# EdwardsLabProjects/sequence-alignment-tools

Measured on AMD Instinct MI355X. Metric: Gbases/s scanned, 100k×20-mer primers k≤2, 3 Gbp DB at 1/2/4/8 GPUs, higher is better.
Workload: dtype u32

## Files before the change

### sequence-alignment-tools_amd/csrc/pm_bits.h

```cpp
#pragma once
#include <cstdint>
#include <utility>

#include <hip/hip_runtime.h>

namespace pm {

namespace {

template <int... Is, typename F>
__device__ __forceinline__ void static_each(std::integer_sequence<int, Is...>, F &&f) { (f(std::integral_constant<int, Is>()), ...); }
template <int N, typename F>
__device__ __forceinline__ void static_for(F &&f) { static_each(std::make_integer_sequence<int, N>(), f); }

template <int O>
__device__ __forceinline__ uint32_t bits_at(uint32_t w0) {
  static_assert(O >= 0 && O < 32, "offset");
  if constexpr (O == 0) return w0;
  else return w0 >> O;
}
template <int O, typename... W>
__device__ __forceinline__ uint32_t bits_at(uint32_t w0, uint32_t w1, W... more) {
  static_assert(O >= 0, "offset");
  if constexpr (O == 0) return w0;
  else if constexpr (O < 32) return __builtin_amdgcn_alignbit(w1, w0, O);
  else return bits_at<O - 32>(w1, more...);
}

template <bool NT = false>
__device__ __forceinline__ uint32_t load_packed(const uint32_t *packed, int64_t npacked, int64_t pos) {
  const int64_t i = pos >> 4;
  if (pos < 0 || i >= npacked) return 0u;
  return NT ? __builtin_nontemporal_load(packed + i) : packed[i];
}

}

}
```

### sequence-alignment-tools_amd/csrc/pm_pair.hip

```cpp
#include "pm_bits.h"
#include "pm_internal.h"
#include "pm_pair.h"
#include "pm_verify.h"
#include "pm_workmap.h"

#include <algorithm>
#include <cstring>
#include <thread>
#include <type_traits>
#include <utility>

namespace pm {

namespace {

constexpr int WAVES = PAIR_WAVES;
constexpr uint32_t F20 = 0xfffffu;
constexpr uint32_t WHAT_REST = 8u, WHAT_ALL = 16u;
__device__ __host__ __forceinline__ uint64_t slot_pack(uint32_t o1, uint32_t o2, uint32_t o3, bool walk) {
  return (uint64_t)o1 | ((uint64_t)o2 << 20) | ((uint64_t)o3 << 40) | ((uint64_t)(walk ? 8 : 0) << 60);
}

struct PairArgs {
  const uint8_t *text;
  int64_t n, begin, end;
  const uint32_t *packed;
  int64_t npacked;
  int64_t chunk0, chunk_len;
  int nchunks, ncombos, group;
  int work_map;
  int k, eos_code, debug;
  int stride;
  int fa[PAIR_MAX_COMBOS], fb[PAIR_MAX_COMBOS];
  const uint32_t *image;
  const uint2 *slots;
  const uint32_t *row_base;
  const uint32_t *first_pat, *order;
  const uint32_t *olist;
  uint32_t first_off[PAIR_MAX_COMBOS];
  uint32_t np;
  const uint2 *pat40;
  const uint8_t *pat_len;
  const uint32_t *pat_id;
  const uint8_t *pat_codes;
  const uint32_t *pat_zone;
  int viol_level;
  pm_hit *out;
  unsigned long long *counter;
  unsigned long long cap;
  uint4 *susp;
  unsigned long long *susp_count;
  unsigned long long susp_cap;
  uint64_t *seed_out;
  unsigned long long *seed_count;
  unsigned long long seed_cap;
  unsigned long long *stats;
};

typedef __attribute__((address_space(3))) uint32_t lds_u32;
typedef uint32_t u32x4 __attribute__((ext_vector_type(4)));
typedef uint32_t u32x2 __attribute__((ext_vector_type(2)));
typedef __attribute__((address_space(3))) u32x4 lds_u128;
__device__ __forceinline__ lds_u128 *lds128(uint32_t addr) { return reinterpret_cast<lds_u128 *>((uintptr_t)addr); }
__device__ __forceinline__ lds_u32 *lds32(uint32_t addr) { return reinterpret_cast<lds_u32 *>((uintptr_t)addr); }

__device__ __host__ __forceinline__ uint32_t field_of(uint64_t W, int j) { return (uint32_t)(W >> (10 * j)) & 0x3ffu; }
__device__ __host__ __forceinline__ void other_fields(int a, int b, int *c, int *d) {
  int o[2], t = 0;
  for (int j = 0; j < 4; ++j) if (j != a && j != b) o[t++] = j;
  *c = o[0]; *d = o[1];
}


template <int OFF>
__device__ __forceinline__ uint32_t wbits(uint32_t wlo, uint32_t whi) {
  static_assert(OFF >= 0 && OFF < 48, "window offset");
  if constexpr (OFF == 0) return wlo;
  else if constexpr (OFF < 32) return __builtin_amdgcn_alignbit(whi, wlo, OFF);
  else return whi >> (OFF - 32);
}
template <int NB, int T>
__device__ __forceinline__ uint32_t mism(uint32_t p, uint32_t wlo, uint32_t whi) {
  static_assert(T >= -2 && T + NB <= 22, "text base outside the window");
  const uint32_t x = p ^ wbits<2 * (T + 2)>(wlo, whi);
  return (x | (x >> 1)) & (NB == 5 ? 0x155u : 0x55555u);
}
enum { REG_L = 0, REG_M = 1, REG_R = 2 };
template <int NB>
__device__ __forceinline__ bool two_deletions(uint32_t lowm, uint32_t midm, uint32_t highm) {
  const int lo = __builtin_ctz(lowm | (1u << (2 * NB)));
  const int hi = 31 - __builtin_clz(highm | 1u);
  const uint32_t between = ((1u << hi) - 1u) & ~((2u << lo) - 1u);
  return (midm & between) == 0;
}
template <int KIND, int NB, int T0, int BASE, int DSP, int BUDGET>
__device__ __forceinline__ int region_cost(uint32_t p, uint32_t wlo, uint32_t whi) {
  const uint32_t m0 = mism<NB, T0 + BASE>(p, wlo, whi);
  if constexpr (KIND == REG_M) {
    if constexpr (DSP == 0) {
      int c = __popc(m0);
      if constexpr (BUDGET >= 2) {
        const int up = 1 + max(1, __popc(m0 & mism<NB, T0 + 1>(p, wlo, whi))), dn = 1 + max(1, __popc(m0 & mism<NB, T0 - 1>(p, wlo, whi)));
        c = min(c, min(up, dn));
      }
      return c;
    }
    else if constexpr (DSP == 1) return 1 + __popc(m0 & mism<NB, T0 - 1>(p, wlo, whi));
    else if constexpr (DSP == -1) return max(1, __popc(m0 & mism<NB, T0 + 1>(p, wlo, whi)));
    else if constexpr (DSP == 2) return 2 + __popc(m0 & mism<NB, T0 - 1>(p, wlo, whi) & mism<NB, T0 - 2>(p, wlo, whi));
    else return two_deletions<NB>(mism<NB, T0 + 2>(p, wlo, whi), mism<NB, T0 + 1>(p, wlo, whi), m0) ? 2 : 9;
  } else {
    int c = __popc(m0);
    if constexpr (BUDGET >= 1) {
      const uint32_t rp1 = mism<NB, T0 + BASE + 1>(p, wlo, whi), rn1 = mism<NB, T0 + BASE - 1>(p, wlo, whi);
      const uint32_t mp1 = m0 & rp1, mn1 = m0 & rn1;
      const int up = __popc(mp1), dn = __popc(mn1);
      c = min(c, KIND == REG_R ? min(1 + up, max(1, dn)) : min(max(1, up), 1 + dn));
      if constexpr (BUDGET >= 2) {
        const uint32_t rp2 = mism<NB, T0 + BASE + 2>(p, wlo, whi), rn2 = mism<NB, T0 + BASE - 2>(p, wlo, whi);
        if constexpr (KIND == REG_R) {
          const int ins2 = 2 + __popc(mp1 & rp2);
          c = min(c, min(ins2, two_deletions<NB>(m0, rn1, rn2) ? 2 : 9));
        } else {
          const int ins2 = 2 + __popc(mn1 & rn2);
          c = min(c, min(ins2, two_deletions<NB>(rp2, rp1, m0) ? 2 : 9));
        }
      }
    }
    return c;
  }
}
template <int A, int B, int DSP, bool LOOSE = false>
__device__ __forceinline__ int edit_cost(uint32_t o, uint32_t wlo, uint32_t whi) {
  constexpr int C = (A != 0 && B != 0) ? 0 : ((A != 1 && B != 1) ? 1 : 2);
  constexpr int D = (A != 3 && B != 3) ? 3 : ((A != 2 && B != 2) ? 2 : 1);
  constexpr int AD = DSP < 0 ? -DSP : DSP, BUD = 2 - AD;
  constexpr int BUD2 = LOOSE && DSP == 0 ? 1 : BUD;
  static_assert(B > A + 1 || DSP == 0, "adjacent key fields are not displaced");
  if constexpr (A == 0 && B == 1) return region_cost<REG_R, 10, 10, 0, 0, BUD>(o, wlo, whi);
  else if constexpr (A == 2 && B == 3) return region_cost<REG_L, 10, 0, 0, 0, BUD>(o, wlo, whi);
  else if constexpr (A == 0 && B == 3) return region_cost<REG_M, 10, 5, 0, DSP, BUD>(o, wlo, whi);
  else {
    int c1, c2;
    if constexpr (A == 1 && B == 2) {
      c1 = region_cost<REG_L, 5, 0, 0, 0, BUD2>(o, wlo, whi);
      c2 = region_cost<REG_R, 5, 15, 0, 0, BUD2>(o >> 10, wlo, whi);
    }
    else if constexpr (A == 0 && B == 2) {
      c1 = region_cost<REG_M, 5, 5, 0, DSP, BUD2>(o, wlo, whi);
      c2 = region_cost<REG_R, 5, 15, 0, 0, BUD2>(o >> 10, wlo, whi);
    }
    else {
      static_assert(A == 1 && B == 3 && C == 0 && D == 2, "fields");
      c1 = region_cost<REG_L, 5, 0, -DSP, 0, BUD2>(o, wlo, whi);
      c2 = region_cost<REG_M, 5, 10, 0, DSP, BUD2>(o >> 10, wlo, whi);
    }
    if constexpr (LOOSE && DSP == 0) return min(c1, c2) == 0 ? 0 : c1 + c2;
    else return c1 + c2;
  }
}
template <int A, int B, int DSP>
__device__ __forceinline__ uint32_t edit_key(uint32_t wlo, uint32_t whi) {
  return (wbits<4 + 10 * A - 2 * DSP>(wlo, whi) & 0x3ffu) | ((wbits<4 + 10 * B>(wlo, whi) & 0x3ffu) << 10);
}
template <typename F>
__device__ __forceinline__ void edit_variant(int v, F &&f) {
  using std::integral_constant;
  switch (v) {
    case 0: f(integral_constant<int, 0>(), integral_constant<int, 1>(), integral_constant<int, 0>()); break;
    case 1: f(integral_constant<int, 0>(), integral_constant<int, 2>(), integral_constant<int, -1>()); break;
    case 2: f(integral_constant<int, 0>(), integral_constant<int, 2>(), integral_constant<int, 0>()); break;
    case 3: f(integral_constant<int, 0>(), integral_constant<int, 2>(), integral_constant<int, 1>()); break;
    case 4: f(integral_constant<int, 0>(), integral_constant<int, 3>(), integral_constant<int, -2>()); break;
    case 5: f(integral_constant<int, 0>(), integral_constant<int, 3>(), integral_constant<int, -1>()); break;
    case 6: f(integral_constant<int, 0>(), integral_constant<int, 3>(), integral_constant<int, 0>()); break;
    case 7: f(integral_constant<int, 0>(), integral_constant<int, 3>(), integral_constant<int, 1>()); break;
    case 8: f(integral_constant<int, 0>(), integral_constant<int, 3>(), integral_constant<int, 2>()); break;
    case 9: f(integral_constant<int, 1>(), integral_constant<int, 2>(), integral_constant<int, 0>()); break;
    case 10: f(integral_constant<int, 1>(), integral_constant<int, 3>(), integral_constant<int, -1>()); break;
    case 11: f(integral_constant<int, 1>(), integral_constant<int, 3>(), integral_constant<int, 0>()); break;
    case 12: f(integral_constant<int, 1>(), integral_constant<int, 3>(), integral_constant<int, 1>()); break;
    case 13: f(integral_constant<int, 2>(), integral_constant<int, 3>(), integral_constant<int, 0>()); break;
    default: break;
  }
}
__device__ __host__ __forceinline__ int edit_variant_table(int var) { return var == 0 ? 0 : (var <= 3 ? 1 : (var <= 8 ? 2 : (var == 9 ? 3 : (var <= 12 ? 4 : 5)))); }


__device__ __forceinline__ void pair_resolve(const PairArgs &a, const VerifyStage &vs, int combo, uint32_t rank, uint32_t what, uint32_t wo, int64_t p, pm_hit *first, bool *have) {
  const uint32_t *fp = a.first_pat + a.first_off[combo];
  const uint32_t *ord = a.order + (size_t)combo * a.np;
  const uint32_t *ol = a.olist + (size_t)combo * a.np;
  const uint32_t t0 = fp[rank], t1 = fp[rank + 1];
  pm_hit hh;
  auto take = [&](bool ok) __attribute__((always_inline)) {
    const bool extra = ok && *have;
    if (ok && !*have) { *first = hh; *have = true; }
    pair_emit(a, vs, extra, hh);
  };
  for (uint32_t j = 0; j < 3; ++j)
    take(((what >> j) & 1u) && t0 + j < t1 && pair_verify<5>(a, combo, p, ord[t0 + j], &hh));
  if (what & (WHAT_REST | WHAT_ALL)) {
    for (uint32_t t = t0 + ((what & WHAT_ALL) ? 0u : 3u); t < t1; ++t)
      take(sym_distance(ol[t] ^ wo) <= a.k && pair_verify<5>(a, combo, p, ord[t], &hh));
  }
}

__global__ __launch_bounds__(256) void pm_pair_verify(PairArgs a) {
  unsigned long long n = *a.susp_count;
  if (n > a.susp_cap) n = a.susp_cap;
  verify_staged(a, n, [&](unsigned long long i, const VerifyStage &vs, pm_hit *first) __attribute__((always_inline)) {
    bool have = false;
    const uint4 r = a.susp[i];
    const uint64_t pw = ((uint64_t)r.w << 32) | r.z;
    if (r.x != 0xffffffffu) {
      const int combo = (int)((pw >> 40) & 7u);
      const uint32_t key = r.x, wo = r.y, row = key & 0x7fffu, bit = key >> 15;
      const uint32_t wd = a.image[(size_t)combo * PAIR_BITMAP_WORDS + row];
      if ((wd >> bit) & 1u) {
        const uint32_t lr = (uint32_t)__popc(wd & ((1u << bit) - 1u));
        const uint32_t rank = a.row_base[(size_t)combo * (PAIR_BITMAP_WORDS + 1) + row] + lr;
        uint32_t what = WHAT_ALL;
        if (lr < (uint32_t)a.stride - 1u) {
          const uint2 sl = a.slots[((size_t)combo * PAIR_BITMAP_WORDS + row) * (size_t)a.stride + lr];
          const uint64_t S = ((uint64_t)sl.y << 32) | sl.x;
          what = (sym_distance(((uint32_t)S ^ wo) & F20) <= a.k ? 1u : 0u) | (sym_distance(((uint32_t)(S >> 20) ^ wo) & F20) <= a.k ? 2u : 0u) |
                 (sym_distance(((uint32_t)(S >> 40) ^ wo) & F20) <= a.k ? 4u : 0u) | ((sl.y >> 31) ? WHAT_REST : 0u);
        }
        pair_resolve(a, vs, combo, rank, what, wo, (int64_t)(pw & 0xffffffffffull), first, &have);
      }
    }
    return have && !(a.debug & 16);
  });
}

template <int A, int B, int DSP = 0, int FLOOR = 0>
__device__ __forceinline__ void pair_scan_body(const PairArgs &a, const int combo, const int cj, const int variant = 0) {
  constexpr int C = (A != 0 && B != 0) ? 0 : ((A != 1 && B != 1) ? 1 : 2);
  constexpr int D = (A != 3 && B != 3) ? 3 : ((A != 2 && B != 2) ? 2 : 1);
  static_assert(A < B && C < D && C != A && C != B && D != A && D != B, "fields");
  const int lane = threadIdx.x & 63;
  const int wave = __builtin_amdgcn_readfirstlane((int)(threadIdx.x >> 6));
  const int64_t sub = a.chunk_len / WAVES;
  const int64_t ws = (a.chunk0 + cj) * a.chunk_len + (int64_t)wave * sub;
  int64_t own_lo = ws > a.begin ? ws : a.begin;
  int64_t own_hi = ws + sub;
  if (own_hi > a.end) own_hi = a.end;
  if (own_hi > a.n) own_hi = a.n;
  if (own_lo < 19) own_lo = 19;
  if (own_lo >= own_hi) return;

  const uint32_t stride = (uint32_t)a.stride, kmax = stride - 1u;
  const char *slots = reinterpret_cast<const char *>(a.slots + (size_t)combo * PAIR_BITMAP_WORDS * stride);
  uint32_t carry1, carry2;
  {
    const uint32_t pk = load_packed(a.packed, a.npacked, ws - 32 + 16 * (lane & 1));
    carry2 = __builtin_amdgcn_readlane(pk, 0);
    carry1 = __builtin_amdgcn_readlane(pk, 1);
  }
  const uint32_t QB = PAIR_BITMAP_WORDS * 4 + (uint32_t)wave * (PAIR_QUEUE * 16);
  int qn = 0;
  uint32_t keep = 0;

  const int64_t pre_hi = FLOOR == 3 ? own_hi + 1024 : own_hi;
  uint32_t q0 = load_packed(a.packed, a.npacked, ws + 16 * lane);
  uint32_t q1 = ws + 1024 < pre_hi ? load_packed(a.packed, a.npacked, ws + 1024 + 16 * lane) : 0u;
  uint32_t q2 = ws + 2048 < pre_hi ? load_packed(a.packed, a.npacked, ws + 2048 + 16 * lane) : 0u;
  uint32_t q3 = ws + 3072 < pre_hi ? load_packed(a.packed, a.npacked, ws + 3072 + 16 * lane) : 0u;
  const uint32_t *pk_wave = a.packed + (ws >> 4);
  uint32_t pf_idx = 4096u / 16u + (uint32_t)lane;

  const int negk1 = -(a.k + 1);

  unsigned long long blk_at = 0;
  uint32_t blk_left = 0, blk_next = 0;
  auto flush = [&]() __attribute__((always_inline)) {
    int done = 0;
    while (done < qn) {
      if (blk_left == 0) {
        const uint32_t want = max((uint32_t)(qn - done), blk_next);
        unsigned long long base = 0;
        if (lane == 0) base = atomicAdd(a.susp_count, (unsigned long long)want);
        blk_at = ((unsigned long long)__builtin_amdgcn_readfirstlane((uint32_t)(base >> 32)) << 32) | __builtin_amdgcn_readfirstlane((uint32_t)base);
        blk_left = want;
        blk_next = min(2u * max(want, 64u), 4096u);
      }
      const int take = min(qn - done, (int)blk_left);
      for (int e = lane; e < take; e += 64) {
        const u32x4 q = *lds128(QB + 16 * (uint32_t)(done + e));
        const uint64_t pw = (uint64_t)(ws + q.z) | ((uint64_t)(FLOOR == 3 ? variant : combo) << 40);
        if (blk_at + (unsigned long long)e < a.susp_cap) a.susp[blk_at + (unsigned long long)e] = make_uint4(q.x, q.y, (uint32_t)pw, (uint32_t)(pw >> 32));
      }
      blk_at += (unsigned long long)take; blk_left -= (uint32_t)take; done += take;
    }
    qn = 0;
  };
  auto give_back = [&]() __attribute__((always_inline)) {
    for (uint32_t e = (uint32_t)lane; e < blk_left; e += 64)
      if (blk_at + e < a.susp_cap) a.susp[blk_at + e] = make_uint4(0xffffffffu, 0xffffffffu, 0xffffffffu, 0xffffffffu);
    blk_left = 0;
  };
  auto enqueue = [&](bool mine, uint32_t key, uint32_t wo, uint32_t prel) __attribute__((always_inline)) {
    const unsigned long long bal = __ballot(mine);
    if (bal == 0) return;
    if (a.debug & 1) { keep ^= key; return; }
    if (mine) {
      const int s_ = qn + (int)__builtin_amdgcn_mbcnt_hi((uint32_t)(bal >> 32), __builtin_amdgcn_mbcnt_lo((uint32_t)bal, 0));
      u32x4 q;
      q.x = key; q.y = wo; q.z = prel; q.w = 0;
      *lds128(QB + 16 * (uint32_t)s_) = q;
    }
    qn += __popcll(bal);
    if (qn >= 64) flush();
  };

  auto key_of = [&](auto WIN, uint32_t prev2, uint32_t prev1, uint32_t cur) __attribute__((always_inline)) -> uint32_t {
    constexpr int I = decltype(WIN)::value;
    const uint32_t X = bits_at<2 * I + 26 + 10 * A - 2 - 2 * DSP>(prev2, prev1, cur);
    if constexpr (B == A + 1 && DSP == 0) return X;
    else { const uint32_t Y = bits_at<2 * I + 26 + 10 * B - 12>(prev2, prev1, cur); return (X & 0xffcu) | (Y & ~0xffcu); }
  };

#ifndef PM_PAIR_NR
#define PM_PAIR_NR 6
#endif
  constexpr int NR = PM_PAIR_NR;
  static_assert(NR % 2 == 0 && NR >= 4 && NR <= 12, "ring size");
  uint32_t P = 0;
  uint32_t pu1 = 0, pu2 = 0, pu3 = 0, cu1 = 0, cu2 = 0, cu3 = 0;
  uint32_t tagbase = 0xfffffff0u;
  u32x2 e_sl[NR];
  uint32_t e_key[NR], e_wo[NR], e_rel[NR], e_okm[NR], e_wd[NR];
  uint32_t e_hi[FLOOR >= 2 ? NR : 1];
  for (int d = 0; d < (FLOOR >= 2 ? NR : 1); ++d) e_hi[d] = 0;
#pragma unroll
  for (int d = 0; d < NR; ++d) { e_sl[d].x = 0; e_sl[d].y = 0; e_key[d] = e_wo[d] = e_rel[d] = e_okm[d] = e_wd[d] = 0; }
  uint32_t m5v, f20v, rowmask;
  asm volatile("v_mov_b32 %0, 0x55555\n v_mov_b32 %1, 0xfffff\n v_mov_b32 %2, 0x7fff" : "=v"(m5v), "=v"(f20v), "=v"(rowmask));

  auto round = [&](auto PHASE) __attribute__((always_inline)) {
    constexpr int PH = decltype(PHASE)::value, LD = (PH + NR - 1) % NR;
    if constexpr (FLOOR == 3) {
      const uint32_t lo = e_wo[PH], hi = e_hi[PH];
      const int d1 = edit_cost<A, B, DSP, true>(e_sl[PH].x & f20v, lo, hi) - 3;
      const int d2 = edit_cost<A, B, DSP, true>(__builtin_amdgcn_alignbit(e_sl[PH].y, e_sl[PH].x, 20) & f20v, lo, hi) - 3;
      const bool susp = (int)(((uint32_t)(d1 | d2) | e_sl[PH].y) & e_okm[PH]) < 0;
      enqueue(susp, lo, hi, ((e_rel[PH] >> 4) << 10) + 16u * (uint32_t)lane + (e_rel[PH] & 15u));
    } else if constexpr (FLOOR == 2) {
      constexpr int OC = 4 + 10 * C;
      const uint32_t lo = e_wo[PH], hi = e_hi[PH];
      uint32_t T[5];
      static_for<5>([&](auto SI) __attribute__((always_inline)) { constexpr int si = decltype(SI)::value; T[si] = __builtin_amdgcn_alignbit(hi, lo, OC + 2 * (si - 2)) & f20v; });
      auto score = [&](uint32_t o) __attribute__((always_inline)) -> int {
        uint32_t m[5];
        static_for<5>([&](auto SI) __attribute__((always_inline)) { constexpr int si = decltype(SI)::value; const uint32_t x = o ^ T[si]; m[si] = (x | (x >> 1)) & m5v; });
        const int c0 = __popc(m[2]), c1 = __popc(m[2] & m[3]) + 1, c1n = __popc(m[2] & m[1]) + 1;
        const int c2 = __popc(m[2] & m[3] & m[4]) + 2, c2n = __popc(m[2] & m[1] & m[0]) + 2;
        return min(min(c0, min(c1, c1n)), min(c2, c2n)) - 3;
      };
      const int d1 = score(e_sl[PH].x & f20v), d2 = score(__builtin_amdgcn_alignbit(e_sl[PH].y, e_sl[PH].x, 20) & f20v);
      const bool susp = (int)(((uint32_t)(d1 | d2) | e_sl[PH].y) & e_okm[PH]) < 0;
      enqueue(susp, e_key[PH], lo, ((e_rel[PH] >> 4) << 10) + 16u * (uint32_t)lane + (e_rel[PH] & 15u));
    } else {
      const uint32_t w = e_wo[PH];
      const uint32_t x1 = e_sl[PH].x ^ w, x2 = __builtin_amdgcn_alignbit(e_sl[PH].y, e_sl[PH].x, 20) ^ w, x3 = (e_sl[PH].y >> 8) ^ w;
      const int d1 = __popc((x1 | (x1 >> 1)) & m5v) + negk1;
      const int d2 = __popc((x2 | (x2 >> 1)) & m5v) + negk1;
      const int d3 = __popc((x3 | (x3 >> 1)) & m5v) + negk1;
      const bool susp = (int)(((uint32_t)(d1 | d2 | d3) | e_sl[PH].y) & e_okm[PH]) < 0;
      enqueue(susp, e_key[PH], w, ((e_rel[PH] >> 4) << 10) + 16u * (uint32_t)lane + (e_rel[PH] & 15u));
    }
    {
      const uint32_t bit = e_key[LD] >> 15;
      const uint32_t lr = min((uint32_t)__popc(__builtin_amdgcn_ubfe(e_wd[LD], 0, bit)), kmax);
      const uint32_t off = (__umul24(e_key[LD] & rowmask, stride) + lr) << 3;
      e_sl[LD] = *reinterpret_cast<const u32x2 *>(slots + off);
    }
    {
      uint32_t i;
      asm("v_ffbl_b32 %0, %1" : "=v"(i) : "v"(P));
      P &= P - 1u;
      const uint32_t okm = ~i;
      const bool cb = (i & 16u) != 0;
      const uint32_t j2 = i + i;
      const uint32_t u1 = cb ? cu1 : pu1, u2 = cb ? cu2 : pu2, u3 = cb ? cu3 : pu3;
      const uint32_t wlo = __builtin_amdgcn_alignbit(u2, u1, j2), whi = __builtin_amdgcn_alignbit(u3, u2, j2);
      auto from = [&](int O) __attribute__((always_inline)) -> uint32_t { return O == 0 ? wlo : (O == 10 ? wlo >> 10 : __builtin_amdgcn_alignbit(whi, wlo, 20)); };
      uint32_t key, wo;
      if constexpr (FLOOR != 0) {
        constexpr int OA = 4 + 10 * A - 2 * DSP, OB = 4 + 10 * B - 10, OCC = 4 + 10 * C, ODD = 4 + 10 * D - 10;
        key = (__builtin_amdgcn_alignbit(whi, wlo, OA) & 0x3ffu) | (__builtin_amdgcn_alignbit(whi, wlo, OB) & 0xffc00u);
        if constexpr (FLOOR >= 2) { wo = wlo; e_hi[PH] = whi; }
        else wo = (__builtin_amdgcn_alignbit(whi, wlo, OCC) & 0x3ffu) | (__builtin_amdgcn_alignbit(whi, wlo, ODD) & 0xffc00u);
      } else {
      if constexpr (B == A + 1) key = from(10 * A) & f20v; else key = (from(10 * A) & 0x3ffu) | (from(10 * B - 10) & 0xffc00u);
      if constexpr (D == C + 1) wo = from(10 * C) & f20v; else wo = (from(10 * C) & 0x3ffu) | (from(10 * D - 10) & 0xffc00u);
      }
      key &= (uint32_t)((int)okm >> 31);
      e_key[PH] = key; e_wo[PH] = wo; e_okm[PH] = okm;
      e_rel[PH] = tagbase + i;
      e_wd[PH] = *lds32((key & rowmask) << 2);
    }
  };
  int ph = 0;
  int quiet = NR + 1;
  auto two_rounds = [&]() __attribute__((always_inline)) {
    bool done = false;
    static_for<NR / 2>([&](auto Q) __attribute__((always_inline)) {
      constexpr int q = decltype(Q)::value;
      if (!done && ph == q) {
        round(std::integral_constant<int, 2 * q>()); round(std::integral_constant<int, 2 * q + 1>());
        ph = q + 1 == NR / 2 ? 0 : q + 1;
        done = true;
      }
    });
  };

  const bool stats = (a.debug & 32) != 0 && a.stats != nullptr;
  uint32_t st_blocks = 0, st_rounds = 0, st_hits = 0;
  int64_t bb = ws;
  const int rmin = (a.debug >> 8) & 15 ? (a.debug >> 8) & 15 : 2;
  while (bb < own_hi) {
    const uint32_t cur = q0;
    q0 = q1; q1 = q2; q2 = q3;
    if (bb + 4096 < pre_hi) q3 = pk_wave[pf_idx];
    pf_idx += 64u;
    const uint32_t prev1 = __builtin_amdgcn_update_dpp(carry1, cur, 0x138, 0xf, 0xf, false);
    const uint32_t prev2 = __builtin_amdgcn_update_dpp(carry2, prev1, 0x138, 0xf, 0xf, false);
    carry2 = __builtin_amdgcn_readlane(cur, 62);
    carry1 = __builtin_amdgcn_readlane(cur, 63);
    uint32_t own = 0xffffu;
    if (bb < own_lo || bb + 1024 > own_hi) {
      const int64_t pbase = bb + 16 * lane;
      const int64_t lo = own_lo - pbase, hi = own_hi - pbase;
      const uint32_t l = lo <= 0 ? 0u : (lo >= 16 ? 16u : (uint32_t)lo), hh = hi <= 0 ? 0u : (hi >= 16 ? 16u : (uint32_t)hi);
      own = ((1u << hh) - 1u) & ~((1u << l) - 1u);
    }
    uint32_t acc = 0;
    {
      uint32_t ks[16], wd[16];
      static_for<16>([&](auto WIN) __attribute__((always_inline)) {
        constexpr int I = decltype(WIN)::value;
        ks[I] = key_of(WIN, prev2, prev1, cur);
        wd[I] = *lds32(ks[I] & 0x1fffcu);
      });
      static_for<16>([&](auto WIN) __attribute__((always_inline)) {
        constexpr int I = decltype(WIN)::value;
        acc = __builtin_amdgcn_alignbit(wd[I] >> ((ks[I] >> 17) & 31u), acc, 1);
      });
    }
    P |= acc & (own << 16);
    if (stats) { st_hits += (uint32_t)__popc(acc & (own << 16)); ++st_blocks; }
    constexpr int WB = FLOOR != 0 ? 22 : 26;
    cu1 = __builtin_amdgcn_alignbit(prev1, prev2, WB); cu2 = __builtin_amdgcn_alignbit(cur, prev1, WB); cu3 = cur >> WB;
    if constexpr (FLOOR == 3) {
      const uint32_t nfirst = __builtin_amdgcn_readfirstlane(q0);
      const uint32_t nxt = __builtin_amdgcn_update_dpp(nfirst, cur, 0x130, 0xf, 0xf, false);
      cu3 |= nxt << 10;
    }
    if (__ballot(P != 0)) quiet = 0;
    if (quiet <= NR) {
      int r = 0;
      do { two_rounds(); r += 2; } while (r < rmin || __ballot((P & 0xffffu) != 0));
      quiet += r;
      st_rounds += (uint32_t)r;
    }
    P >>= 16; pu1 = cu1; pu2 = cu2; pu3 = cu3; tagbase += 16u;
    bb += 1024;
  }
  while (__ballot(P != 0)) two_rounds();
  for (int d = 0; d < NR / 2 + 1; ++d) two_rounds();
  if (keep == 0x9e3779b9u) a.susp[0] = make_uint4(keep, 0, 0, 0);
  flush();
  give_back();
  if (stats) {
    for (int o = 32; o > 0; o >>= 1) st_hits += (uint32_t)__shfl_xor((int)st_hits, o);
    if (lane == 0) { atomicAdd(a.stats, (unsigned long long)st_blocks); atomicAdd(a.stats + 1, (unsigned long long)st_rounds); atomicAdd(a.stats + 2, (unsigned long long)st_hits); }
  }
}

__device__ __forceinline__ bool pair_block_item(const PairArgs &a, int *combo, int *cj) {
  if (a.work_map == PAIR_MAP_XCD_SUPERCHUNK) pair_xcd_superchunk_item((int)blockIdx.x, a.nchunks, a.ncombos, a.group, combo, cj);
  else if (a.work_map == PAIR_MAP_XCD) pair_xcd_item((int)blockIdx.x, a.nchunks, a.ncombos, combo, cj);
  else pair_superchunk_item((int)blockIdx.x, a.nchunks, a.ncombos, a.group, combo, cj);
  return *cj < a.nchunks && *combo < a.ncombos;
}

__global__ __launch_bounds__(PAIR_THREADS) void pm_pair_scan(PairArgs a) {
  extern __shared__ uint32_t lds[];
  int combo, cj;
  if (!pair_block_item(a, &combo, &cj)) return;
  {
    const u32x4 *src = reinterpret_cast<const u32x4 *>(a.image + (size_t)combo * PAIR_BITMAP_WORDS);
    u32x4 *dst = reinterpret_cast<u32x4 *>(lds);
    for (int i = threadIdx.x; i < PAIR_BITMAP_WORDS / 4; i += PAIR_THREADS) dst[i] = src[i];
  }
  __syncthreads();
  const int fa = a.fa[combo], fb = a.fb[combo];
  switch (fa * 4 + fb) {
    case 1: pair_scan_body<0, 1>(a, combo, cj); break;
    case 2: pair_scan_body<0, 2>(a, combo, cj); break;
    case 3: pair_scan_body<0, 3>(a, combo, cj); break;
    case 6: pair_scan_body<1, 2>(a, combo, cj); break;
    case 7: pair_scan_body<1, 3>(a, combo, cj); break;
    case 11: pair_scan_body<2, 3>(a, combo, cj); break;
    default: break;
  }
}

template <int FLOOR>
__global__ __launch_bounds__(PAIR_THREADS) void pm_pair_edit_scan(PairArgs a) {
  extern __shared__ uint32_t lds[];
  int var, cj;
  if (!pair_block_item(a, &var, &cj)) return;
  const int table = edit_variant_table(var);
  {
    const u32x4 *src = reinterpret_cast<const u32x4 *>(a.image + (size_t)table * PAIR_BITMAP_WORDS);
    u32x4 *dst = reinterpret_cast<u32x4 *>(lds);
    for (int i = threadIdx.x; i < PAIR_BITMAP_WORDS / 4; i += PAIR_THREADS) dst[i] = src[i];
  }
  __syncthreads();
  switch (var) {
    case 0: pair_scan_body<0, 1, 0, FLOOR>(a, table, cj, 0); break;
    case 1: pair_scan_body<0, 2, -1, FLOOR>(a, table, cj, 1); break;
    case 2: pair_scan_body<0, 2, 0, FLOOR>(a, table, cj, 2); break;
    case 3: pair_scan_body<0, 2, 1, FLOOR>(a, table, cj, 3); break;
    case 4: pair_scan_body<0, 3, -2, FLOOR>(a, table, cj, 4); break;
    case 5: pair_scan_body<0, 3, -1, FLOOR>(a, table, cj, 5); break;
    case 6: pair_scan_body<0, 3, 0, FLOOR>(a, table, cj, 6); break;
    case 7: pair_scan_body<0, 3, 1, FLOOR>(a, table, cj, 7); break;
    case 8: pair_scan_body<0, 3, 2, FLOOR>(a, table, cj, 8); break;
    case 9: pair_scan_body<1, 2, 0, FLOOR>(a, table, cj, 9); break;
    case 10: pair_scan_body<1, 3, -1, FLOOR>(a, table, cj, 10); break;
    case 11: pair_scan_body<1, 3, 0, FLOOR>(a, table, cj, 11); break;
    case 12: pair_scan_body<1, 3, 1, FLOOR>(a, table, cj, 12); break;
    case 13: pair_scan_body<2, 3, 0, FLOOR>(a, table, cj, 13); break;
    default: break;
  }
}

constexpr int ESTAGE = 2048;
constexpr int EWORK = 3072;
__global__ __launch_bounds__(256) void pm_pair_edit_resolve(PairArgs a) {
  __shared__ uint64_t s_rec[ESTAGE];
  __shared__ uint4 s_susp[256];
  __shared__ uint32_t s_work[EWORK];
  __shared__ uint32_t s_t0[256];
  __shared__ unsigned long long s_base;
  __shared__ uint32_t s_fill, s_valid, s_full, s_nwork;
  unsigned long long n = *a.susp_count;
  if (n > a.susp_cap) n = a.susp_cap;
  const unsigned long long stride = (unsigned long long)gridDim.x * blockDim.x;
  const int lane = threadIdx.x & 63;
  if (threadIdx.x == 0) { s_fill = 0; s_valid = (uint32_t)ESTAGE; s_nwork = 0; }
  __syncthreads();
  auto emit = [&](bool ok, uint64_t rec) __attribute__((always_inline)) {
    const unsigned long long bal = __ballot(ok);
    if (bal == 0) return;
    const int leader = __ffsll((long long)bal) - 1;
    const uint32_t cnt = (uint32_t)__popcll(bal), mine = (uint32_t)__popcll(bal & ((1ull << lane) - 1ull));
    uint32_t pos = 0;
    if (lane == leader) pos = atomicAdd(&s_fill, cnt);
    pos = __builtin_amdgcn_readlane(pos, leader);
    if (pos + cnt <= (uint32_t)ESTAGE) { if (ok) s_rec[pos + mine] = rec; return; }
    unsigned long long base = 0;
    if (lane == leader) { atomicMin(&s_valid, pos); base = atomicAdd(a.seed_count, (unsigned long long)cnt); }
    const uint32_t blo = __builtin_amdgcn_readlane((uint32_t)base, leader), bhi = __builtin_amdgcn_readlane((uint32_t)(base >> 32), leader);
    if (ok) { const unsigned long long o = (((unsigned long long)bhi << 32) | blo) + mine; if (o < a.seed_cap) a.seed_out[o] = rec; }
  };
  auto flush = [&]() __attribute__((always_inline)) {
    __syncthreads();
    const uint32_t cnt = min(s_fill, s_valid);
    __syncthreads();
    if (threadIdx.x == 0) { s_base = cnt ? atomicAdd(a.seed_count, (unsigned long long)cnt) : 0ull; s_fill = 0; s_valid = (uint32_t)ESTAGE; }
    __syncthreads();
    for (uint32_t i = threadIdx.x; i < cnt; i += blockDim.x) if (s_base + i < a.seed_cap) a.seed_out[s_base + i] = s_rec[i];
    __syncthreads();
  };
  auto item = [&](uint32_t wlo, uint32_t whi, int var, uint64_t pos40, uint32_t t, bool live) __attribute__((always_inline)) {
    bool ok = false;
    uint64_t rec = 0;
    if (live) {
      const int table = edit_variant_table(var);
      const uint32_t o = a.olist[(size_t)table * a.np + t];
      int c = 9;
      edit_variant(var, [&](auto A_, auto B_, auto D_) __attribute__((always_inline)) { c = edit_cost<decltype(A_)::value, decltype(B_)::value, decltype(D_)::value>(o, wlo, whi); });
      ok = c <= 2;
      if (ok) rec = ((uint64_t)a.order[(size_t)table * a.np + t] << 40) | pos40;
    }
    emit(ok, rec);
  };
  for (unsigned long long base = (unsigned long long)blockIdx.x * blockDim.x; base < n; base += stride) {
    const unsigned long long i = base + threadIdx.x;
    uint32_t t0 = 0, t1 = 0;
    uint4 r = make_uint4(0, 0, 0, 0xffffffffu);
    if (i < n) r = a.susp[i];
    if (r.w != 0xffffffffu) {
      const int var = (int)((r.w >> 8) & 15u);
      uint32_t key = 0;
      edit_variant(var, [&](auto A_, auto B_, auto D_) __attribute__((always_inline)) { key = edit_key<decltype(A_)::value, decltype(B_)::value, decltype(D_)::value>(r.x, r.y); });
      const int table = edit_variant_table(var);
      const uint32_t row = key & 0x7fffu, bit = key >> 15;
      const uint32_t wd = a.image[(size_t)table * PAIR_BITMAP_WORDS + row];
      if ((wd >> bit) & 1u) {
        const uint32_t rank = a.row_base[(size_t)table * (PAIR_BITMAP_WORDS + 1) + row] + (uint32_t)__popc(wd & ((1u << bit) - 1u));
        const uint32_t *fp = a.first_pat + a.first_off[table];
        t0 = fp[rank]; t1 = fp[rank + 1];
      }
    }
    s_susp[threadIdx.x] = r;
    s_t0[threadIdx.x] = t0;
    const uint32_t len = t1 - t0;
    uint32_t at = len ? atomicAdd(&s_nwork, len) : 0u;
    uint32_t q = 0;
    for (; q < len && at + q < (uint32_t)EWORK; ++q) s_work[at + q] = ((uint32_t)threadIdx.x << 24) | q;
    __syncthreads();
    const uint32_t nw = min(s_nwork, (uint32_t)EWORK);
    for (uint32_t w0 = 0; w0 < nw; w0 += blockDim.x) {
      const uint32_t w = w0 + threadIdx.x;
      const bool live = w < nw;
      const uint32_t it = live ? s_work[w] : 0u;
      const uint4 sr = s_susp[it >> 24];
      item(sr.x, sr.y, (int)((sr.w >> 8) & 15u), ((uint64_t)(sr.w & 0xffu) << 32) | sr.z, s_t0[it >> 24] + (it & 0xffffffu), live);
    }
    {
      uint32_t t = t0 + q;
      while (__ballot(t < t1)) { item(r.x, r.y, (int)((r.w >> 8) & 15u), ((uint64_t)(r.w & 0xffu) << 32) | r.z, t, t < t1); if (t < t1) ++t; }
    }
    __syncthreads();
    if (threadIdx.x == 0) { s_full = s_fill > (uint32_t)(ESTAGE - 1024); s_nwork = 0; }
    __syncthreads();
    if (s_full) flush();
  }
  flush();
}

}


std::string pair_build(const std::vector<Pattern> &pats, const std::vector<uint32_t> &ids, const Alphabet &alpha, int k,
                       int eos_code, PairTables *out, int stride_knob, int slot_patterns) {
  const size_t SP = slot_patterns == 2 ? 2 : 3;
  PairTables &t = *out;
  t = PairTables();
  if (k < 1 || k > 2) return "the pair plan is built for k = 1 and k = 2";
  const bool norm = alpha.nch['A'] == 0 && alpha.nch['C'] == 1 && alpha.nch['G'] == 2 && alpha.nch['T'] == 3;
  const bool ascii = alpha.size == 256 && alpha.nch['A'] == 'A' && alpha.nch['C'] == 'C' && alpha.nch['G'] == 'G' && alpha.nch['T'] == 'T';
  if (!norm && !ascii) return "stream alphabet is neither A,C,G,T-normalized nor raw ASCII";
  t.ascii = ascii && !norm;
  t.k = k;
  t.eos_code = (eos_code >= 0 && eos_code < 256) ? eos_code : -1;
  auto base2 = [&](unsigned char ch) -> int {
    switch (ch) { case 'A': return 0; case 'C': return 1; case 'G': return t.ascii ? 3 : 2; case 'T': return t.ascii ? 2 : 3; }
    return -1;
  };
  const size_t np = pats.size();
  if (np == 0) return "no patterns";
  if (np >= ((size_t)1 << 30)) return "too many patterns";
  t.pat40.resize(np); t.pat_len.resize(np); t.pat_id.resize(np); t.pat_codes.assign(np * 32, 0); t.pat_zone.assign(np, 0);
  for (size_t j = 0; j < np; ++j) {
    const std::string &s = pats[j].s;
    const int L = (int)s.size();
    if (L < 20 || L > 32) return "the pair plan needs patterns of 20..32 characters";
    uint64_t w = 0;
    for (int i = 0; i < 20; ++i) {
      const int b2 = base2((unsigned char)s[L - 20 + i]);
      if (b2 < 0) return "pattern with characters other than A,C,G,T";
      w |= (uint64_t)b2 << (2 * i);
    }
    for (int i = 0; i < L; ++i) {
      if (base2((unsigned char)s[i]) < 0) return "pattern with characters other than A,C,G,T";
      t.pat_codes[j * 32 + i] = (uint8_t)alpha.nch[(unsigned char)s[i]];
    }
    t.pat40[j] = w; t.pat_len[j] = (uint8_t)L; t.pat_id[j] = ids[j];
    {
      const int es = std::max(0, std::min(L, pats[j].esb)), ee = std::max(0, std::min(L, pats[j].eeb));
      uint32_t z = 0;
      for (int i = 0; i < L; ++i) if (i < es || i >= L - ee) z |= 1u << i;
      t.pat_zone[j] = z;
    }
    t.maxlen = std::max(t.maxlen, L);
  }
  if (k == 1) { t.ncombos = 2; t.fa[0] = 0; t.fb[0] = 1; t.fa[1] = 2; t.fb[1] = 3; }
  else { t.ncombos = 0; for (int x = 0; x < 4; ++x) for (int y = x + 1; y < 4; ++y) { t.fa[t.ncombos] = x; t.fb[t.ncombos] = y; ++t.ncombos; } }
  const int C = t.ncombos;
  t.stride = stride_knob >= 2 && stride_knob <= 33 ? stride_knob : (np <= 230000 ? 12 : (np <= 300000 ? 14 : 16));
  const size_t ST = (size_t)t.stride, KMAX = ST - 1;
  t.image.assign((size_t)C * PAIR_BITMAP_WORDS, 0);
  t.order.assign((size_t)C * np, 0);
  t.olist.assign((size_t)C * np, 0);
  t.slots.assign((size_t)C * PAIR_BITMAP_WORDS * ST, 0);
  t.row_base.assign((size_t)C * (PAIR_BITMAP_WORDS + 1), 0);
  std::vector<std::vector<uint32_t>> fp(C);
  auto build_combo = [&](int ci) {
    const int fa = t.fa[ci], fb = t.fb[ci];
    int fc, fd;
    other_fields(fa, fb, &fc, &fd);
    std::vector<uint64_t> srt(np);
    for (size_t j = 0; j < np; ++j) {
      const uint32_t key = field_of(t.pat40[j], fa) | (field_of(t.pat40[j], fb) << 10);
      const uint32_t bitpos = ((key & 0x7fffu) << 5) | (key >> 15);
      srt[j] = ((uint64_t)bitpos << 32) | (uint64_t)j;
    }
    std::sort(srt.begin(), srt.end());
    uint32_t *img = &t.image[(size_t)ci * PAIR_BITMAP_WORDS];
    uint32_t *ord = &t.order[(size_t)ci * np];
    uint32_t *ol = &t.olist[(size_t)ci * np];
    uint64_t *slot = &t.slots[(size_t)ci * PAIR_BITMAP_WORDS * ST];
    uint32_t *rb = &t.row_base[(size_t)ci * (PAIR_BITMAP_WORDS + 1)];
    std::vector<uint32_t> &f = fp[ci];
    f.reserve(np + 1);
    for (size_t r = 0; r < (size_t)PAIR_BITMAP_WORDS; ++r) slot[r * ST + KMAX] = slot_pack(0, 0, 0, true);
    uint32_t cur_row = 0, in_row = 0;
    for (size_t j = 0; j < np;) {
      const uint32_t bitpos = (uint32_t)(srt[j] >> 32);
      size_t j2 = j;
      while (j2 < np && (uint32_t)(srt[j2] >> 32) == bitpos) ++j2;
      const uint32_t row = bitpos >> 5;
      while (cur_row < row) { rb[++cur_row] = (uint32_t)f.size(); in_row = 0; }
      img[row] |= 1u << (bitpos & 31u);
      f.push_back((uint32_t)j);
      uint32_t o[3] = {0, 0, 0};
      for (size_t q = j; q < j2; ++q) {
        const uint32_t pi = (uint32_t)srt[q];
        ord[q] = pi;
        ol[q] = field_of(t.pat40[pi], fc) | (field_of(t.pat40[pi], fd) << 10);
        if (q - j < SP) o[q - j] = field_of(t.pat40[pi], fc) | (field_of(t.pat40[pi], fd) << 10);
      }
      for (size_t q = std::min(j2 - j, SP); q < 3; ++q) o[q] = o[0];
      if (in_row < KMAX) slot[(size_t)row * ST + in_row] = slot_pack(o[0], o[1], o[2], j2 - j > SP);
      ++in_row;
      j = j2;
    }
    while (cur_row < (uint32_t)PAIR_BITMAP_WORDS) rb[++cur_row] = (uint32_t)f.size();
    f.push_back((uint32_t)np);
  };
  if (np * (size_t)C < 20000) for (int ci = 0; ci < C; ++ci) build_combo(ci);
  else {
    std::vector<std::thread> th;
    for (int ci = 0; ci < C; ++ci) th.emplace_back([&, ci]() { build_combo(ci); });
    for (std::thread &x : th) x.join();
  }
  for (int ci = 0; ci < C; ++ci) {
    t.first_off[ci] = t.first_pat.size();
    t.first_pat.insert(t.first_pat.end(), fp[ci].begin(), fp[ci].end());
  }
  return "";
}

hipError_t pair_upload(const PairTables &t, PairDevice *d, hipStream_t st) {
  pair_free(d);
  d->k = t.k; d->maxlen = t.maxlen; d->ncombos = t.ncombos; d->eos_code = t.eos_code; d->ascii = t.ascii; d->np = t.pat40.size(); d->stride = t.stride;
  for (int c = 0; c < PAIR_MAX_COMBOS; ++c) { d->fa[c] = t.fa[c]; d->fb[c] = t.fb[c]; d->first_off[c] = t.first_off[c]; }
  auto up = [&](const void *src, size_t bytes, void **dst) -> hipError_t {
    hipError_t e = hipMalloc(dst, bytes ? bytes : 16);
    if (e != hipSuccess) return e;
    return bytes ? hipMemcpyAsync(*dst, src, bytes, hipMemcpyHostToDevice, st) : hipSuccess;
  };
  hipError_t e;
  if ((e = up(t.image.data(), t.image.size() * 4, (void **)&d->image)) != hipSuccess) return e;
  if ((e = up(t.slots.data(), t.slots.size() * 8, (void **)&d->slots)) != hipSuccess) return e;
  if ((e = up(t.row_base.data(), t.row_base.size() * 4, (void **)&d->row_base)) != hipSuccess) return e;
  if ((e = up(t.first_pat.data(), t.first_pat.size() * 4, (void **)&d->first_pat)) != hipSuccess) return e;
  if ((e = up(t.order.data(), t.order.size() * 4, (void **)&d->order)) != hipSuccess) return e;
  if ((e = up(t.olist.data(), t.olist.size() * 4, (void **)&d->olist)) != hipSuccess) return e;
  if ((e = up(t.pat40.data(), t.pat40.size() * 8, (void **)&d->pat40)) != hipSuccess) return e;
  if ((e = up(t.pat_len.data(), t.pat_len.size(), (void **)&d->pat_len)) != hipSuccess) return e;
  if ((e = up(t.pat_id.data(), t.pat_id.size() * 4, (void **)&d->pat_id)) != hipSuccess) return e;
  if ((e = up(t.pat_codes.data(), t.pat_codes.size(), (void **)&d->pat_codes)) != hipSuccess) return e;
  if ((e = up(t.pat_zone.data(), t.pat_zone.size() * 4, (void **)&d->pat_zone)) != hipSuccess) return e;
  hipFuncAttributes fa;
  if ((e = hipFuncGetAttributes(&fa, reinterpret_cast<const void *>(pm_pair_scan))) != hipSuccess) return e;
  if (fa.sharedSizeBytes != 0) return hipErrorInvalidConfiguration;
  if ((e = hipFuncSetAttribute(reinterpret_cast<const void *>(pm_pair_scan), hipFuncAttributeMaxDynamicSharedMemorySize, PAIR_LDS_BYTES)) != hipSuccess) return e;
  return hipStreamSynchronize(st);
}

void pair_free(PairDevice *d) {
  void *ptrs[] = {d->image, d->slots, d->row_base, d->first_pat, d->order, d->olist, d->pat_id, d->pat40, d->pat_len, d->pat_codes, d->pat_zone};
  for (void *p : ptrs) if (p) (void)hipFree(p);
  *d = PairDevice();
}

ScanGeometry pair_geometry(const PairDevice &d, int64_t begin, int64_t end) {
  ScanGeometry g;
  int64_t chunk = 1 << 19;
  const int64_t range = end - begin;
  if (range / ((int64_t)1 << 21) * d.ncombos >= 256 * 16) chunk = (int64_t)1 << 21;
  else if (range / ((int64_t)1 << 20) * d.ncombos >= 256 * 16) chunk = (int64_t)1 << 20;
  if (d.knobs.seed_chunk >= 1024 * WAVES) chunk = d.knobs.seed_chunk / (1024 * WAVES) * (1024 * WAVES);
  g.seg_len = chunk;
  const int64_t c_lo = begin / chunk, c_hi = end > begin ? (end - 1) / chunk : c_lo - 1;
  g.nseg = (int)(c_hi - c_lo + 1);
  g.threads = PAIR_THREADS;
  g.blocks = g.nseg * d.ncombos;
  g.work_map = g.nseg >= PAIR_XCD_MIN_CHUNKS ? PAIR_MAP_XCD_SUPERCHUNK : PAIR_MAP_SUPERCHUNK;
  if (d.knobs.pair_map >= 0) g.work_map = d.knobs.pair_map;
  return g;
}

hipError_t pair_launch(const PairDevice &d, const uint8_t *d_text, const uint32_t *d_packed, int64_t n, int64_t begin, int64_t end,
                       pm_hit *d_out, unsigned long long *d_counter, uint64_t cap, void *d_susp, unsigned long long *d_susp_count, uint64_t susp_cap,
                       hipStream_t st, ScanGeometry *geo_out, unsigned long long *d_stats, int floor_mode,
                       uint64_t *seed_out, unsigned long long *seed_count, uint64_t seed_cap) {
  if (!d_packed) return hipErrorInvalidValue;
  if (end > n) end = n;
  if (floor_mode && (d.k != 2 || d.ncombos != 6)) return hipErrorInvalidValue;
  if (floor_mode == 3 && (!seed_out || !seed_count)) return hipErrorInvalidValue;
  ScanGeometry g = pair_geometry(d, begin, end);
  if (floor_mode) {
    g.blocks = g.nseg * 14;
    if (d.knobs.pair_map < 0) g.work_map = PAIR_MAP_SUPERCHUNK;
  }
  if (geo_out) *geo_out = g;
  if (g.blocks <= 0 || d.np == 0) return hipSuccess;
  PairArgs a;
  memset(&a, 0, sizeof(a));
  a.text = d_text; a.n = n; a.begin = begin; a.end = end;
  a.packed = d_packed; a.npacked = (n + 15) / 16;
  a.chunk_len = g.seg_len; a.chunk0 = begin / g.seg_len; a.nchunks = g.nseg; a.ncombos = d.ncombos;
  a.group = 256;
  if (d.knobs.seed_group > 0) a.group = d.knobs.seed_group;
  a.work_map = g.work_map;
  a.k = d.k; a.eos_code = d.eos_code;
  a.debug = d.knobs.seed_debug;
  for (int c = 0; c < PAIR_MAX_COMBOS; ++c) { a.fa[c] = d.fa[c]; a.fb[c] = d.fb[c]; a.first_off[c] = (uint32_t)d.first_off[c]; }
  a.stride = d.stride;
  a.image = d.image; a.slots = reinterpret_cast<const uint2 *>(d.slots); a.row_base = d.row_base; a.first_pat = d.first_pat; a.order = d.order; a.olist = d.olist;
  a.np = (uint32_t)d.np;
  a.pat40 = reinterpret_cast<const uint2 *>(d.pat40); a.pat_len = d.pat_len; a.pat_id = d.pat_id; a.pat_codes = d.pat_codes; a.pat_zone = d.pat_zone; a.viol_level = d.viol_level;
  a.out = d_out; a.counter = d_counter; a.cap = cap;
  if (!d_susp || !d_susp_count) return hipErrorInvalidValue;
  a.susp = reinterpret_cast<uint4 *>(d_susp); a.susp_count = d_susp_count; a.susp_cap = susp_cap;
  a.stats = d_stats;
  a.seed_out = seed_out; a.seed_count = seed_count; a.seed_cap = seed_cap;
  if (floor_mode) {
    a.ncombos = 14;
    hipError_t fe;
    if (floor_mode == 1) {
      if ((fe = hipFuncSetAttribute(reinterpret_cast<const void *>(pm_pair_edit_scan<1>), hipFuncAttributeMaxDynamicSharedMemorySize, PAIR_LDS_BYTES)) != hipSuccess) return fe;
      hipLaunchKernelGGL(pm_pair_edit_scan<1>, dim3(g.blocks), dim3(PAIR_THREADS), PAIR_LDS_BYTES, st, a);
    } else if (floor_mode == 2) {
      if ((fe = hipFuncSetAttribute(reinterpret_cast<const void *>(pm_pair_edit_scan<2>), hipFuncAttributeMaxDynamicSharedMemorySize, PAIR_LDS_BYTES)) != hipSuccess) return fe;
      hipLaunchKernelGGL(pm_pair_edit_scan<2>, dim3(g.blocks), dim3(PAIR_THREADS), PAIR_LDS_BYTES, st, a);
    } else {
      if ((fe = hipFuncSetAttribute(reinterpret_cast<const void *>(pm_pair_edit_scan<3>), hipFuncAttributeMaxDynamicSharedMemorySize, PAIR_LDS_BYTES)) != hipSuccess) return fe;
      hipLaunchKernelGGL(pm_pair_edit_scan<3>, dim3(g.blocks), dim3(PAIR_THREADS), PAIR_LDS_BYTES, st, a);
      if ((fe = hipGetLastError()) != hipSuccess) return fe;
      hipLaunchKernelGGL(pm_pair_edit_resolve, dim3(16384), dim3(256), 0, st, a);
    }
    return hipGetLastError();
  }
  hipLaunchKernelGGL(pm_pair_scan, dim3(g.blocks), dim3(PAIR_THREADS), PAIR_LDS_BYTES, st, a);
  hipError_t ce = hipGetLastError();
  if (ce != hipSuccess) return ce;
  hipLaunchKernelGGL(pm_pair_verify, dim3(32768), dim3(256), 0, st, a);
  return hipGetLastError();
}

}
```

Baseline: 216.3.

## Restructure pair scan into a continuous round pipeline with a deeper text prefetch queue

Replaces the per-block loop, which dispatched two_rounds through a runtime phase switch, with a state machine. Verify rounds now run in a statically unrolled ring, and block boundaries (load next word, compute bitmap hits) are handled at ring edges, so the software pipeline of slot loads stays full across blocks and drain stages. The prefetch queue depth now scales with NR/2+1, and late-landing loads are joined into the queue through asm barriers. The aim is to remove phase-dispatch branching and pipeline bubbles at block transitions, at the cost of much more complex control flow and higher register pressure.

```diff
diff --git a/sequence-alignment-tools_amd/csrc/pm_bits.h b/sequence-alignment-tools_amd/csrc/pm_bits.h
--- a/sequence-alignment-tools_amd/csrc/pm_bits.h
+++ b/sequence-alignment-tools_amd/csrc/pm_bits.h
@@ -12,6 +12,10 @@
 __device__ __forceinline__ void static_each(std::integer_sequence<int, Is...>, F &&f) { (f(std::integral_constant<int, Is>()), ...); }
 template <int N, typename F>
 __device__ __forceinline__ void static_for(F &&f) { static_each(std::make_integer_sequence<int, N>(), f); }
+template <int... Is, typename F>
+__device__ __forceinline__ bool static_all_each(std::integer_sequence<int, Is...>, F &&f) { return (f(std::integral_constant<int, Is>()) && ...); }
+template <int N, typename F>
+__device__ __forceinline__ bool static_all(F &&f) { return static_all_each(std::make_integer_sequence<int, N>(), f); }
 
 template <int O>
 __device__ __forceinline__ uint32_t bits_at(uint32_t w0) {
diff --git a/sequence-alignment-tools_amd/csrc/pm_pair.hip b/sequence-alignment-tools_amd/csrc/pm_pair.hip
--- a/sequence-alignment-tools_amd/csrc/pm_pair.hip
+++ b/sequence-alignment-tools_amd/csrc/pm_pair.hip
@@ -263,12 +263,7 @@
   uint32_t keep = 0;
 
   const int64_t pre_hi = FLOOR == 3 ? own_hi + 1024 : own_hi;
-  uint32_t q0 = load_packed(a.packed, a.npacked, ws + 16 * lane);
-  uint32_t q1 = ws + 1024 < pre_hi ? load_packed(a.packed, a.npacked, ws + 1024 + 16 * lane) : 0u;
-  uint32_t q2 = ws + 2048 < pre_hi ? load_packed(a.packed, a.npacked, ws + 2048 + 16 * lane) : 0u;
-  uint32_t q3 = ws + 3072 < pre_hi ? load_packed(a.packed, a.npacked, ws + 3072 + 16 * lane) : 0u;
   const uint32_t *pk_wave = a.packed + (ws >> 4);
-  uint32_t pf_idx = 4096u / 16u + (uint32_t)lane;
 
   const int negk1 = -(a.k + 1);
 
@@ -374,6 +369,7 @@
       const uint32_t bit = e_key[LD] >> 15;
       const uint32_t lr = min((uint32_t)__popc(__builtin_amdgcn_ubfe(e_wd[LD], 0, bit)), kmax);
       const uint32_t off = (__umul24(e_key[LD] & rowmask, stride) + lr) << 3;
+      asm volatile("" : : "v"(e_sl[LD]));
       e_sl[LD] = *reinterpret_cast<const u32x2 *>(slots + off);
     }
     {
@@ -402,29 +398,36 @@
       e_wd[PH] = *lds32((key & rowmask) << 2);
     }
   };
-  int ph = 0;
   int quiet = NR + 1;
-  auto two_rounds = [&]() __attribute__((always_inline)) {
-    bool done = false;
-    static_for<NR / 2>([&](auto Q) __attribute__((always_inline)) {
-      constexpr int q = decltype(Q)::value;
-      if (!done && ph == q) {
-        round(std::integral_constant<int, 2 * q>()); round(std::integral_constant<int, 2 * q + 1>());
-        ph = q + 1 == NR / 2 ? 0 : q + 1;
-        done = true;
-      }
-    });
-  };
 
   const bool stats = (a.debug & 32) != 0 && a.stats != nullptr;
   uint32_t st_blocks = 0, st_rounds = 0, st_hits = 0;
   int64_t bb = ws;
   const int rmin = (a.debug >> 8) & 15 ? (a.debug >> 8) & 15 : 2;
-  while (bb < own_hi) {
-    const uint32_t cur = q0;
-    q0 = q1; q1 = q2; q2 = q3;
-    if (bb + 4096 < pre_hi) q3 = pk_wave[pf_idx];
-    pf_idx += 64u;
+  constexpr int PD = NR / 2 + 1;
+  uint32_t q[PD], land[NR / 2];
+  static_for<PD>([&](auto I) __attribute__((always_inline)) {
+    constexpr int i = decltype(I)::value;
+    q[i] = i == 0 || ws + 1024 * i < pre_hi ? load_packed(a.packed, a.npacked, ws + 1024 * i + 16 * lane) : 0u;
+  });
+  static_for<NR / 2>([&](auto I) __attribute__((always_inline)) { land[decltype(I)::value] = 0; });
+  int qfill = PD;
+  uint32_t landed = 0;
+  uint32_t pf_idx = (uint32_t)PD * 64u + (uint32_t)lane;
+  auto q_take = [&]() __attribute__((always_inline)) -> uint32_t {
+    const uint32_t cur = q[0];
+    static_for<PD - 1>([&](auto I) __attribute__((always_inline)) { constexpr int i = decltype(I)::value; q[i] = q[i + 1]; });
+    --qfill;
+    return cur;
+  };
+  auto q_join = [&](uint32_t w) __attribute__((always_inline)) {
+    static_for<PD>([&](auto I) __attribute__((always_inline)) {
+      constexpr int i = decltype(I)::value;
+      if (qfill == i) { const uint32_t from = w; uint32_t to; asm volatile("v_mov_b32 %0, %1" : "=v"(to) : "v"(from)); q[i] = to; }
+    });
+    ++qfill;
+  };
+  auto block_begin = [&](const uint32_t cur) __attribute__((always_inline)) {
     const uint32_t prev1 = __builtin_amdgcn_update_dpp(carry1, cur, 0x138, 0xf, 0xf, false);
     const uint32_t prev2 = __builtin_amdgcn_update_dpp(carry2, prev1, 0x138, 0xf, 0xf, false);
     carry2 = __builtin_amdgcn_readlane(cur, 62);
@@ -454,22 +457,69 @@
     constexpr int WB = FLOOR != 0 ? 22 : 26;
     cu1 = __builtin_amdgcn_alignbit(prev1, prev2, WB); cu2 = __builtin_amdgcn_alignbit(cur, prev1, WB); cu3 = cur >> WB;
     if constexpr (FLOOR == 3) {
-      const uint32_t nfirst = __builtin_amdgcn_readfirstlane(q0);
+      const uint32_t nfirst = __builtin_amdgcn_readfirstlane(q[0]);
       const uint32_t nxt = __builtin_amdgcn_update_dpp(nfirst, cur, 0x130, 0xf, 0xf, false);
       cu3 |= nxt << 10;
     }
-    if (__ballot(P != 0)) quiet = 0;
-    if (quiet <= NR) {
-      int r = 0;
-      do { two_rounds(); r += 2; } while (r < rmin || __ballot((P & 0xffffu) != 0));
-      quiet += r;
-      st_rounds += (uint32_t)r;
-    }
+  };
+  int r = 0;
+  int rlim = rmin;
+  int stage = 0;
+  auto block_end = [&]() __attribute__((always_inline)) {
+    quiet += r; if (stage == 0) st_rounds += (uint32_t)r;
     P >>= 16; pu1 = cu1; pu2 = cu2; pu3 = cu3; tagbase += 16u;
-    bb += 1024;
-  }
-  while (__ballot(P != 0)) two_rounds();
-  for (int d = 0; d < NR / 2 + 1; ++d) two_rounds();
+    bb += 1024; r = 0;
+  };
+  bool leave = false;
+  auto edge = [&](auto Q) __attribute__((always_inline)) -> bool {
+    constexpr int e = decltype(Q)::value;
+    if (e == 0 && leave) return false;
+    if (landed & (1u << e)) { q_join(land[e]); landed &= ~(1u << e); }
+    if (leave) return true;
+    if (r < rlim || __ballot((P & 0xffffu) != 0)) return true;
+    block_end();
+    if (bb < own_hi) {
+      const uint32_t cur = q_take();
+      if (bb + 1024 * PD < pre_hi) land[e] = pk_wave[pf_idx];
+      pf_idx += 64u; landed |= 1u << e;
+      block_begin(cur);
+      if (__ballot(P != 0)) quiet = 0;
+      leave = quiet > NR;
+    }
+    else if (stage == 0 && __ballot(P != 0)) { stage = 1; rlim = 0; }
+    else if (stage < 2) { stage = 2; rlim = NR; }
+    else { stage = 3; leave = true; }
+    return true;
+  };
+  while (stage < 3) {
+    for (;;) {
+      if (bb >= own_hi) { stage = 3; break; }
+      const uint32_t cur = q_take();
+      if (bb + 1024 * PD < pre_hi) q[PD - 1] = pk_wave[pf_idx];
+      pf_idx += 64u; ++qfill;
+      block_begin(cur);
+      if (__ballot(P != 0)) quiet = 0;
+      if (quiet <= NR) break;
+      block_end();
+    }
+    if (stage == 3) break;
+    leave = false;
+    { const uint32_t last = q[PD - 1]; asm volatile("" : : "v"(last)); }
+    while (static_all<NR / 2>([&](auto Q) __attribute__((always_inline)) {
+      constexpr int q2 = decltype(Q)::value;
+      if (!edge(Q)) return false;
+      round(std::integral_constant<int, 2 * q2>()); round(std::integral_constant<int, 2 * q2 + 1>());
+      r += 2;
+      return true;
+    })) {}
+    static_for<NR / 2>([&](auto E) __attribute__((always_inline)) {
+      constexpr int e = decltype(E)::value;
+      if (landed & (1u << e)) q_join(land[e]);
+    });
+    landed = 0;
+    r = 0;
+    if (stage < 3) block_end();
+  }
   if (keep == 0x9e3779b9u) a.susp[0] = make_uint4(keep, 0, 0, 0);
   flush();
   give_back();
```

Result: slower. 213.0 (-1.5%).

## Restructure scan loop into phase-unrolled ring state machine with unconditional prefetch

Applied to the files above, without the earlier changes.

Replaces the main scan loop, which dispatched on a runtime ring phase through two_rounds, with an unrolled for(;;) chain of per-phase macros. Each ring pair is compiled with a static phase, and new blocks are taken only when the ring is ready to advance. The prefetch load becomes unconditional, clamping its index to the lane instead of branching, and readfirstlane moves earlier. Both changes aim to remove per-round phase-selection branches and let loads overlap compute. The cost is larger code, goto-based control flow, and tail handling that relies on tagbase and P shift bookkeeping being kept exactly in step.

```diff
diff --git a/sequence-alignment-tools_amd/csrc/pm_pair.hip b/sequence-alignment-tools_amd/csrc/pm_pair.hip
--- a/sequence-alignment-tools_amd/csrc/pm_pair.hip
+++ b/sequence-alignment-tools_amd/csrc/pm_pair.hip
@@ -328,7 +328,7 @@
   static_assert(NR % 2 == 0 && NR >= 4 && NR <= 12, "ring size");
   uint32_t P = 0;
   uint32_t pu1 = 0, pu2 = 0, pu3 = 0, cu1 = 0, cu2 = 0, cu3 = 0;
-  uint32_t tagbase = 0xfffffff0u;
+  uint32_t tagbase = 0xffffffe0u;
   u32x2 e_sl[NR];
   uint32_t e_key[NR], e_wo[NR], e_rel[NR], e_okm[NR], e_wd[NR];
   uint32_t e_hi[FLOOR >= 2 ? NR : 1];
@@ -415,16 +415,25 @@
       }
     });
   };
-
   const bool stats = (a.debug & 32) != 0 && a.stats != nullptr;
   uint32_t st_blocks = 0, st_rounds = 0, st_hits = 0;
   int64_t bb = ws;
   const int rmin = (a.debug >> 8) & 15 ? (a.debug >> 8) & 15 : 2;
-  while (bb < own_hi) {
-    const uint32_t cur = q0;
-    q0 = q1; q1 = q2; q2 = q3;
-    if (bb + 4096 < pre_hi) q3 = pk_wave[pf_idx];
+
+  auto next_word = [&](uint32_t *nfirst) __attribute__((always_inline)) -> uint32_t {
+    uint32_t cur, n0, n1, n2;
+    asm volatile("v_mov_b32 %0, %4\n v_mov_b32 %1, %5\n v_mov_b32 %2, %6\n v_mov_b32 %3, %7"
+                 : "=&v"(cur), "=&v"(n0), "=&v"(n1), "=&v"(n2) : "v"(q0), "v"(q1), "v"(q2), "v"(q3));
+    q0 = n0; q1 = n1; q2 = n2;
+    q3 = pk_wave[bb + 4096 < pre_hi ? pf_idx : (uint32_t)lane];
     pf_idx += 64u;
+    if constexpr (FLOOR == 3) *nfirst = __builtin_amdgcn_readfirstlane(q0);
+    return cur;
+  };
+  auto take_block = [&]() __attribute__((always_inline)) {
+    P >>= 16; pu1 = cu1; pu2 = cu2; pu3 = cu3; tagbase += 16u;
+    uint32_t nfirst = 0;
+    const uint32_t cur = next_word(&nfirst);
     const uint32_t prev1 = __builtin_amdgcn_update_dpp(carry1, cur, 0x138, 0xf, 0xf, false);
     const uint32_t prev2 = __builtin_amdgcn_update_dpp(carry2, prev1, 0x138, 0xf, 0xf, false);
     carry2 = __builtin_amdgcn_readlane(cur, 62);
@@ -454,22 +463,46 @@
     constexpr int WB = FLOOR != 0 ? 22 : 26;
     cu1 = __builtin_amdgcn_alignbit(prev1, prev2, WB); cu2 = __builtin_amdgcn_alignbit(cur, prev1, WB); cu3 = cur >> WB;
     if constexpr (FLOOR == 3) {
-      const uint32_t nfirst = __builtin_amdgcn_readfirstlane(q0);
       const uint32_t nxt = __builtin_amdgcn_update_dpp(nfirst, cur, 0x130, 0xf, 0xf, false);
       cu3 |= nxt << 10;
     }
+    bb += 1024;
     if (__ballot(P != 0)) quiet = 0;
-    if (quiet <= NR) {
-      int r = 0;
-      do { two_rounds(); r += 2; } while (r < rmin || __ballot((P & 0xffffu) != 0));
-      quiet += r;
-      st_rounds += (uint32_t)r;
-    }
-    P >>= 16; pu1 = cu1; pu2 = cu2; pu3 = cu3; tagbase += 16u;
-    bb += 1024;
-  }
-  while (__ballot(P != 0)) two_rounds();
-  for (int d = 0; d < NR / 2 + 1; ++d) two_rounds();
+  };
+
+#define PM_QUIET_BLOCKS(q)                                                                                                   \
+    while (quiet > NR) {                                                                                                     \
+      if (bb >= own_hi) { ph = (q); goto range_end; }                                                                        \
+      take_block();                                                                                                          \
+    }
+#define PM_RING_PAIR(q)                                                                                                      \
+    if constexpr (2 * (q) < NR) {                                                                                            \
+      if (adv) {                                                                                                             \
+        if (bb >= own_hi) { ph = (q); goto range_end; }                                                                      \
+        take_block();                                                                                                        \
+        PM_QUIET_BLOCKS(q)                                                                                                   \
+        r = 0;                                                                                                               \
+      }                                                                                                                      \
+      round(std::integral_constant<int, (2 * (q)) % NR>()); round(std::integral_constant<int, (2 * (q) + 1) % NR>());        \
+      r += 2;                                                                                                                \
+      adv = !(r < rmin || __ballot((P & 0xffffu) != 0));                                                                     \
+      if (adv) { quiet += r; st_rounds += (uint32_t)r; }                                                                     \
+    }
+  {
+    int r = 0;
+    bool adv = false;
+    PM_QUIET_BLOCKS(0)
+    asm volatile("" : : "v"(q0), "v"(q1), "v"(q2), "v"(q3));
+    for (;;) { PM_RING_PAIR(0) PM_RING_PAIR(1) PM_RING_PAIR(2) PM_RING_PAIR(3) PM_RING_PAIR(4) PM_RING_PAIR(5) }
+  }
+#undef PM_RING_PAIR
+#undef PM_QUIET_BLOCKS
+range_end:
+  P >>= 16; pu1 = cu1; pu2 = cu2; pu3 = cu3; tagbase += 16u;
+  for (int d = 0; d < NR / 2 + 1;) {
+    if (!__ballot(P != 0)) ++d;
+    two_rounds();
+  }
   if (keep == 0x9e3779b9u) a.susp[0] = make_uint4(keep, 0, 0, 0);
   flush();
   give_back();
```

New measurement: 215.5 before, 215.3 after. Within noise of the previous version (-0.1%).
